# bailuding/rails

Hardware: AMD Instinct MI355X
Metric: queries/sec, MoL exact top-k over N items (get_top_k_outputs: score + top-k' + id map + seen-id filter) (higher is better)
Workload: dtype f32

## Files before the change

rails_amd/csrc/topk.hip:

```cpp
#include <hip/hip_runtime.h>
#include <stdlib.h>

#include "mol_kernels.h"

namespace mol {

constexpr int kSortCap = 16384;
constexpr int kSortThreads = 1024;
constexpr int kHistThreads = 512;
constexpr int kRadixPasses = 3;
constexpr int kBins = 2048;
__device__ __constant__ int kPassShift[kRadixPasses] = {53, 42, 32};
__device__ __constant__ int kPassBits[kRadixPasses] = {11, 11, 10};

struct SelectState {
  unsigned long long prefix;
  unsigned int need;
  unsigned int done;
  unsigned int count;
  unsigned int pad;
};

__device__ __forceinline__ unsigned int orderable(float f) {
  const unsigned int u = __float_as_uint(f);
// ... 1373 lines not shown
  if (f_invalid && !(k_out <= kFuseMaxK && f_width >= 0 && f_width <= kFuseMaxW && f_k > 0 && f_k <= k_out)) {
    set_error("merge_candidates: the seen-id filter cannot be fused at k = %d, width = %d", k_out, f_width);
    return kErrUnsupported;
  }
  const int64_t count = (int64_t)R * k;
  if (count > kSortCap) { set_error("merge_candidates: R*k = %lld exceeds the in-LDS sort capacity (%d)", (long long)count, kSortCap); return kErrUnsupported; }
  if (ensure_sort_lds() != kOk) return kErrLaunch;
  static DynLdsOnce once;
  if (ensure_dyn_lds(once, reinterpret_cast<const void*>(&merge_candidates_kernel), kSortCap * (int)sizeof(unsigned long long)) != kOk)
    return kErrLaunch;
  const int npad = next_pow2((int)count < 2 ? 2 : (int)count);
  MergeVerdictArgs v{};
  int msg_ld = 2 * k;
  if (verdict) {
    v.default_eps = verdict->default_eps; v.safety = verdict->safety; v.guard = verdict->guard; v.guard_per_row = verdict->guard ? verdict->guard_per_row : 0;
    v.guard_limit = verdict->guard_limit; v.state = verdict->state; v.state_host = verdict->state_host; v.call = verdict->call;
    msg_ld = 2 * k + 2;
  }
  hipLaunchKernelGGL(merge_candidates_kernel, dim3(rows), dim3(kSortThreads), npad * sizeof(unsigned long long), stream, gathered, R,
                     rows, k, k_out, npad, out_scores, out_ids, f_invalid, f_width, f_k, msg_ld, v);
  return hipGetLastError() == hipSuccess ? kOk : kErrLaunch;
}

__global__ __launch_bounds__(kSortThreads) void rescore_select_kernel(const float* __restrict__ exact, int64_t ld,
                                                                      const float* __restrict__ approx,
                                                                      const float* __restrict__ approx_dense, int64_t ld_dense,
                                                                      const int64_t* __restrict__ positions,
                                                                      const int64_t* __restrict__ ids, int n_ranked, int kc, int k, int npad,
                                                                      float margin_eps, float check_eps, int one_sided, float* __restrict__ out_scores,
                                                                      int64_t* __restrict__ out_ids, int* __restrict__ ok,
                                                                      float* __restrict__ stats) {
  extern __shared__ __attribute__((aligned(16))) unsigned long long keys[];
  __shared__ float red_min[kSortThreads / 64], red_err[kSortThreads / 64];
  __shared__ int red_nan[kSortThreads / 64];
  const int row = blockIdx.x;
  float mn = INFINITY, err = 0.0f;
  int bad = 0;
  for (int i = threadIdx.x; i < npad; i += kSortThreads) {
    unsigned long long kv = 0ull;
    if (i < kc) {
      const float e = exact[(int64_t)row * ld + i];
      const int64_t pos = positions[(int64_t)row * kc + i];
      float a;
      if (i < n_ranked) {
        a = approx[(int64_t)row * n_ranked + i];
        kv = ((unsigned long long)orderable(e) << 32) | (unsigned int)(~(unsigned int)pos);
        mn = fminf(mn, a);
      } else {
        a = approx_dense[(int64_t)row * ld_dense + pos];
      }
      const float dd = one_sided ? e - a : fabsf(e - a);
      bad |= !(dd <= check_eps);
      err = fmaxf(err, dd == dd ? dd : INFINITY);
    }
    keys[i] = kv;
  }
#pragma unroll
  for (int o = 32; o > 0; o >>= 1) {
    mn = fminf(mn, __shfl_xor(mn, o, 64));
    err = fmaxf(err, __shfl_xor(err, o, 64));
    bad |= __shfl_xor(bad, o, 64);
  }
  if ((threadIdx.x & 63) == 0) { red_min[threadIdx.x >> 6] = mn; red_err[threadIdx.x >> 6] = err; red_nan[threadIdx.x >> 6] = bad; }
  __syncthreads();
  for (int size = 2; size <= npad; size <<= 1) {
    for (int stride = size >> 1; stride > 0; stride >>= 1) {
      for (int t = threadIdx.x; t < (npad >> 1); t += kSortThreads) {
        const int lo = ((t & ~(stride - 1)) << 1) | (t & (stride - 1));
        const int hi2 = lo | stride;
        const bool desc = ((lo & size) == 0);
        const unsigned long long a = keys[lo], b = keys[hi2];
        if ((a < b) == desc) { keys[lo] = b; keys[hi2] = a; }
      }
      __syncthreads();
    }
  }
  for (int j = threadIdx.x; j < k; j += kSortThreads) {
    const unsigned long long kv = keys[j];
    const int64_t pos = (int64_t)(~(unsigned int)(kv & 0xFFFFFFFFull));
    out_scores[(int64_t)row * k + j] = unorderable((unsigned int)(kv >> 32));
    out_ids[(int64_t)row * k + j] = ids ? ids[pos] : pos;
  }
  if (threadIdx.x == 0) {
    float m = INFINITY, er = 0.0f;
    int b = 0;
    for (int w = 0; w < kSortThreads / 64; ++w) { m = fminf(m, red_min[w]); er = fmaxf(er, red_err[w]); b |= red_nan[w]; }
    const float kth = unorderable((unsigned int)(keys[k - 1] >> 32));
    if (ok) ok[row] = (!b && kth > m + margin_eps) ? 1 : 0;
    if (stats) { stats[2 * row] = er; stats[2 * row + 1] = kth - m; }
  }
}

__global__ __launch_bounds__(256) void rescore_verdict_kernel(const float* __restrict__ row_stats, int rows, float default_eps, float safety,
                                                              const float* __restrict__ guard, int64_t guard_count, float guard_limit,
                                                              float* __restrict__ state) {
  __shared__ float s_err[256], s_gap[256], s_grd[256];
  __shared__ int s_bad[256];
  float err = 0.0f, gap = INFINITY, grd = 0.0f;
  int bad = 0;
  for (int r = threadIdx.x; r < rows; r += 256) {
    const float e = row_stats[2 * r], g = row_stats[2 * r + 1];
    if (!(e == e) || !(g == g)) bad = 1;
    err = fmaxf(err, e);
    gap = fminf(gap, g);
  }
  for (int64_t i = threadIdx.x; i < guard_count; i += 256) {
    const float v = fabsf(guard[i]);
    if (!(v <= guard_limit)) bad = 1;
    grd = fmaxf(grd, v == v ? v : INFINITY);
  }
  s_err[threadIdx.x] = err; s_gap[threadIdx.x] = gap; s_bad[threadIdx.x] = bad; s_grd[threadIdx.x] = grd;
  __syncthreads();
  for (int w = 128; w > 0; w >>= 1) {
    if ((int)threadIdx.x < w) {
      s_err[threadIdx.x] = fmaxf(s_err[threadIdx.x], s_err[threadIdx.x + w]);
      s_gap[threadIdx.x] = fminf(s_gap[threadIdx.x], s_gap[threadIdx.x + w]);
      s_grd[threadIdx.x] = fmaxf(s_grd[threadIdx.x], s_grd[threadIdx.x + w]);
      s_bad[threadIdx.x] |= s_bad[threadIdx.x + w];
    }
    __syncthreads();
  }
  if (threadIdx.x == 0) {
    err = s_err[0]; gap = s_gap[0]; bad = s_bad[0] || !(err < INFINITY);
    float seen = state[0];
    if (!bad) seen = fmaxf(seen, err);
    const float eps = fmaxf(default_eps, safety * seen);
    const int redo = bad || !(gap > eps);
    state[0] = seen;
    reinterpret_cast<int32_t*>(state)[1] = redo;
    state[2] = eps;
    state[3] = bad ? INFINITY : err;
    state[4] = gap;
    state[5] += 1.0f;
    if (redo) state[6] += 1.0f;
    state[7] = fmaxf(state[7], s_grd[0]);
  }
}

int rescore_verdict(const float* row_stats, int rows, float default_eps, float safety, const float* guard, int64_t guard_count, float guard_limit,
                    float* state, hipStream_t stream) {
  hipLaunchKernelGGL(rescore_verdict_kernel, dim3(1), dim3(256), 0, stream, row_stats, rows, default_eps, safety, guard, guard ? guard_count : 0,
                     guard_limit, state);
  return hipGetLastError() == hipSuccess ? kOk : kErrLaunch;
}

__global__ void margin_stats_kernel(const float* __restrict__ kth, int64_t ld, int col, const float* __restrict__ m_max, const float* __restrict__ err_max,
                                    int rows, float* __restrict__ row_stats) {
  const int r = blockIdx.x * blockDim.x + threadIdx.x;
  if (r >= rows) return;
  row_stats[2 * r] = err_max[0];
  row_stats[2 * r + 1] = kth[(int64_t)r * ld + col] - m_max[r];
}
int margin_stats(const float* kth, int64_t ld, int col, const float* m_max, const float* err_max, int rows, float* row_stats, hipStream_t stream) {
  if (rows <= 0) return kOk;
  hipLaunchKernelGGL(margin_stats_kernel, dim3((rows + 255) / 256), dim3(256), 0, stream, kth, ld, col, m_max, err_max, rows, row_stats);
  return hipGetLastError() == hipSuccess ? kOk : kErrLaunch;
}

int rescore_select(const float* exact, int64_t ld, const float* approx, const float* approx_dense, int64_t ld_dense, const int64_t* positions,
                   const int64_t* ids, int rows, int n_ranked, int kc, int k, float margin_eps, float check_eps, int one_sided, float* out_scores,
                   int64_t* out_ids, int* ok, float* stats, hipStream_t stream) {
  if (rows <= 0) return kOk;
  if (kc > kSortCap) { set_error("rescore_select: %d candidates exceed the in-LDS sort capacity (%d)", kc, kSortCap); return kErrUnsupported; }
  static DynLdsOnce once;
  if (ensure_dyn_lds(once, reinterpret_cast<const void*>(&rescore_select_kernel), kSortCap * (int)sizeof(unsigned long long)) != kOk)
    return kErrLaunch;
  const int npad = next_pow2(kc < 2 ? 2 : kc);
  hipLaunchKernelGGL(rescore_select_kernel, dim3(rows), dim3(kSortThreads), npad * sizeof(unsigned long long), stream, exact, ld, approx,
                     approx_dense, ld_dense, positions, ids, n_ranked, kc, k, npad, margin_eps, check_eps, one_sided, out_scores, out_ids, ok, stats);
  return hipGetLastError() == hipSuccess ? kOk : kErrLaunch;
}

__global__ __launch_bounds__(kSortThreads) void sort_rows_i64_kernel(const int64_t* __restrict__ in, int n, int npad,
                                                                    int64_t* __restrict__ out) {
  extern __shared__ __attribute__((aligned(16))) unsigned long long keys[];
  const int row = blockIdx.x;
  if (npad >= 2 * kSortThreads && npad <= 16 * kSortThreads) {
    for (int i = threadIdx.x; i < npad; i += kSortThreads)
      keys[i] = i < n ? ~((unsigned long long)in[(int64_t)row * n + i] ^ 0x8000000000000000ull) : 0ull;
    __syncthreads();
    if (npad == 2 * kSortThreads) block_sort_desc_multi<2>(keys);
    else if (npad == 4 * kSortThreads) block_sort_desc_multi<4>(keys);
    else if (npad == 8 * kSortThreads) block_sort_desc_multi<8>(keys);
    else block_sort_desc_multi<16>(keys);
    for (int i = threadIdx.x; i < n; i += kSortThreads) out[(int64_t)row * n + i] = (int64_t)(~keys[i] ^ 0x8000000000000000ull);
    return;
  }
  for (int i = threadIdx.x; i < npad; i += kSortThreads)
    keys[i] = i < n ? ((unsigned long long)in[(int64_t)row * n + i] ^ 0x8000000000000000ull) : ~0ull;
  __syncthreads();
  for (int size = 2; size <= npad; size <<= 1) {
    for (int stride = size >> 1; stride > 0; stride >>= 1) {
      for (int t = threadIdx.x; t < (npad >> 1); t += kSortThreads) {
        const int lo = ((t & ~(stride - 1)) << 1) | (t & (stride - 1));
        const int hi2 = lo | stride;
        const bool asc = ((lo & size) == 0);
        const unsigned long long a = keys[lo], b = keys[hi2];
        if ((a > b) == asc) { keys[lo] = b; keys[hi2] = a; }
      }
      __syncthreads();
    }
  }
  for (int i = threadIdx.x; i < n; i += kSortThreads) out[(int64_t)row * n + i] = (int64_t)(keys[i] ^ 0x8000000000000000ull);
}

__global__ void mask_sorted_duplicates_kernel(const int64_t* __restrict__ idx, float* __restrict__ scores, int64_t ld,
                                              int rows, int n, float fill) {
  const int64_t i = (int64_t)blockIdx.x * blockDim.x + threadIdx.x;
  if (i >= (int64_t)rows * n) return;
  const int row = (int)(i / n), j = (int)(i - (int64_t)row * n);
  if (j > 0 && idx[i] == idx[i - 1]) scores[(int64_t)row * ld + j] = fill;
}

int sort_rows_i64(const int64_t* in, int rows, int n, int64_t* out, hipStream_t stream) {
  if (rows <= 0 || n <= 0) return kOk;
  if (n > kSortCap) { set_error("sort_rows_i64: n = %d exceeds the in-LDS sort capacity (%d)", n, kSortCap); return kErrUnsupported; }
  static DynLdsOnce once;
  if (ensure_dyn_lds(once, reinterpret_cast<const void*>(&sort_rows_i64_kernel), kSortCap * (int)sizeof(unsigned long long)) != kOk)
    return kErrLaunch;
  const int npad = next_pow2(n < 2 ? 2 : n);
  hipLaunchKernelGGL(sort_rows_i64_kernel, dim3(rows), dim3(kSortThreads), npad * sizeof(unsigned long long), stream, in, n, npad, out);
  return hipGetLastError() == hipSuccess ? kOk : kErrLaunch;
}

int mask_sorted_duplicates(const int64_t* idx, float* scores, int64_t ld, int rows, int n, float fill, hipStream_t stream) {
  const int64_t total = (int64_t)rows * n;
  if (total <= 0) return kOk;
  hipLaunchKernelGGL(mask_sorted_duplicates_kernel, dim3((unsigned)((total + 255) / 256)), dim3(256), 0, stream, idx, scores, ld, rows, n, fill);
  return hipGetLastError() == hipSuccess ? kOk : kErrLaunch;
}

constexpr int kRerankHash = 16384;
constexpr int kRerankMax = 8192;

__global__ __launch_bounds__(1024) void rerank_keys_kernel(const float* __restrict__ scores, int64_t ld, const int64_t* __restrict__ positions, int n,
                                                          int min_unique, unsigned long long* __restrict__ keys, int32_t* __restrict__ flag) {
  extern __shared__ unsigned int rr_tab[];
  const int row = blockIdx.x, tid = threadIdx.x;
  for (int i = tid; i <= kRerankHash; i += 1024) rr_tab[i] = i < kRerankHash ? 0xFFFFFFFFu : 0u;
  __syncthreads();
  unsigned int uniq = 0u;
  for (int c = tid; c < n; c += 1024) {
    const unsigned int p = (unsigned int)positions[(int64_t)row * n + c];
    unsigned int h = (p * 2654435761u) >> 18;
    bool first;
    for (;;) {
      const unsigned int old = atomicCAS(&rr_tab[h], 0xFFFFFFFFu, p);
      if (old == 0xFFFFFFFFu) { first = true; break; }
      if (old == p) { first = false; break; }
      h = (h + 1u) & (unsigned int)(kRerankHash - 1);
    }
    keys[(int64_t)row * n + c] = first ? make_key(scores[(int64_t)row * ld + c], p) : 0ull;
    uniq += first ? 1u : 0u;
  }
#pragma unroll
  for (int o = 32; o > 0; o >>= 1) uniq += (unsigned int)__shfl_xor((int)uniq, o, 64);
  if ((tid & 63) == 0 && uniq) atomicAdd(&rr_tab[kRerankHash], uniq);
  __syncthreads();
  if (tid == 0 && rr_tab[kRerankHash] < (unsigned int)min_unique) *flag = 1;
}

size_t rerank_workspace_bytes(int rows, int n_cand) { return sizeof(unsigned long long) * (size_t)rows * (size_t)n_cand; }

int rerank_topk_filtered(const float* scores, int64_t ld, int rows, int n_cand, int k_prime, const int64_t* positions, const int64_t* ids,
                         const int64_t* invalid, int width, int k, void* ws, size_t ws_bytes, int64_t* out_ids, float* out_scores, int32_t* flag,
                         hipStream_t stream) {
  if (rows <= 0 || k <= 0) return kOk;
  if (n_cand <= 1024 || n_cand > kRerankMax || !topk_can_fuse_filter(n_cand, k_prime, width, k) || k_prime > n_cand) {
    set_error("rerank_topk_filtered: unsupported size (n_cand = %d, k' = %d, width = %d, k = %d)", n_cand, k_prime, width, k);
    return kErrUnsupported;
  }
  if (ws_bytes < rerank_workspace_bytes(rows, n_cand)) { set_error("rerank_topk_filtered: workspace too small"); return kErrNoMem; }
  if (ensure_sort_lds() != kOk) return kErrLaunch;
  static DynLdsOnce once;
  const int lds = (kRerankHash + 16) * (int)sizeof(unsigned int);
  if (ensure_dyn_lds(once, reinterpret_cast<const void*>(&rerank_keys_kernel), lds) != kOk) return kErrLaunch;
  unsigned long long* keys = static_cast<unsigned long long*>(ws);
  hipLaunchKernelGGL(rerank_keys_kernel, dim3(rows), dim3(1024), lds, stream, scores, ld, positions, n_cand, k_prime, keys, flag);
  if (hipGetLastError() != hipSuccess) return kErrLaunch;
  RowSelectArgs b{};
  b.keys_in = keys; b.keys_per_row = n_cand; b.k = k_prime;
  b.ids = ids; b.ids_row_stride = 0; b.out_scores = out_scores; b.out_ids = out_ids;
  b.f_invalid = invalid; b.f_width = width; b.f_k = k;
  return launch_row_select<true>(b, rows, 1, n_cand, stream);
}

int filter_seen(const int64_t* top_ids, const float* top_scores, int rows, int k_prime, const int64_t* invalid,
                int width, int k, int64_t* out_ids, float* out_scores, hipStream_t stream) {
  if (rows <= 0) return kOk;
  if (k > k_prime) { set_error("seen-id filter: k (%d) > k' (%d)", k, k_prime); return kErrInvalid; }
  const size_t lds = sizeof(int64_t) * (size_t)width + (size_t)k_prime + 16;
  if (lds > 60000) { set_error("seen-id filter: k' or width too large for LDS"); return kErrUnsupported; }
  if (k_prime > 1024)
    hipLaunchKernelGGL(filter_seen_kernel<1024>, dim3(rows), dim3(1024), lds, stream, top_ids, top_scores, k_prime, invalid, width, k, out_ids, out_scores);
  else
    hipLaunchKernelGGL(filter_seen_kernel<256>, dim3(rows), dim3(256), lds, stream, top_ids, top_scores, k_prime, invalid, width, k, out_ids, out_scores);
  return hipGetLastError() == hipSuccess ? kOk : kErrLaunch;
}

constexpr int kCandBins = 4096, kCandCoarse = 64, kCandPer = kCandBins / kCandCoarse;
constexpr int kCandThreads = 512;
constexpr int kCandSingleMax = 65536;
constexpr int kCandStage = 2048;

struct CandWs { unsigned int* counts; unsigned int* flags; unsigned int* call; unsigned int* coarse; unsigned int* fine; };
static size_t cand_rows_pad(int rows) { return ((size_t)rows + 3) / 4 * 4; }
static size_t cand_ws_words(int rows) { return cand_rows_pad(rows) * 2 + 8 + (size_t)rows * 4 + (size_t)rows * kCandCoarse + (size_t)rows * kCandBins; }
static CandWs cand_ws(void* ws, int rows) {
  unsigned int* w = static_cast<unsigned int*>(ws);
  const size_t rp = cand_rows_pad(rows);
  CandWs c;
  c.counts = w; c.flags = w + rp; c.call = w + 2 * rp; c.coarse = c.call + 8 + 4 * (size_t)rows; c.fine = c.coarse + (size_t)rows * kCandCoarse;
  return c;
}
size_t candidates_workspace_bytes(int rows) { return cand_ws_words(rows < 1 ? 1 : rows) * sizeof(unsigned int); }

__device__ __forceinline__ int cand_bin(float s, float lo, float scale) {
  float x = (s - lo) * scale;
  x = fminf(fmaxf(x, 0.0f), (float)(kCandBins - 1));
  return (int)x;
}

template <int NT, class F4, class F1>
__device__ __forceinline__ void walk_chunk4(const float* __restrict__ rowp, int64_t begin, int64_t end, F4 f4, F1 f1) {
  int64_t a0 = begin + ((4 - (int64_t)((reinterpret_cast<uintptr_t>(rowp + begin) >> 2) & 3)) & 3);
  if (a0 > end) a0 = end;
  const int64_t nvec = (end - a0) >> 2;
  for (int64_t i = begin + threadIdx.x; i < a0; i += NT) f1(rowp[i], i);
  const float4* body = reinterpret_cast<const float4*>(rowp + a0);
  int64_t v = threadIdx.x;
  for (; v + 3 * NT < nvec; v += 4 * NT) {
    const float4 x0 = body[v], x1 = body[v + NT], x2 = body[v + 2 * NT], x3 = body[v + 3 * NT];
    f4(x0, a0 + 4 * v); f4(x1, a0 + 4 * (v + NT)); f4(x2, a0 + 4 * (v + 2 * NT)); f4(x3, a0 + 4 * (v + 3 * NT));
  }
  for (; v < nvec; v += NT) f4(body[v], a0 + 4 * v);
  for (int64_t i = a0 + 4 * nvec + threadIdx.x; i < end; i += NT) f1(rowp[i], i);
}

__device__ __forceinline__ float cand_threshold_value(int bt, float lo, float scale) {
  if (bt <= 0) return -INFINITY;
  if (cand_bin(INFINITY, lo, scale) < bt) return __uint_as_float(0x7FC00000u);
  if (cand_bin(-INFINITY, lo, scale) >= bt) return -INFINITY;
  unsigned int a = orderable(-INFINITY), b = orderable(INFINITY);
  while (b - a > 1u) {
    const unsigned int mid = a + ((b - a) >> 1);
    if (cand_bin(unorderable(mid), lo, scale) >= bt) b = mid; else a = mid;
  }
  return unorderable(b);
}

template <int NT>
__device__ __forceinline__ void cand_coarse_sums(const unsigned int* h, unsigned int* hc) {
  constexpr int run = kCandBins / NT;
  constexpr int per = kCandPer / run;
  unsigned int s = 0u;
#pragma unroll
  for (int j = 0; j < run; ++j) s += h[threadIdx.x * run + j];
#pragma unroll
  for (int o = 1; o < per; o <<= 1) s += __shfl_xor(s, o, 64);
  if ((threadIdx.x & (per - 1)) == 0) hc[threadIdx.x / per] = s;
}

__device__ __forceinline__ int cand_pick(const unsigned int* coarse, const unsigned int* fine, unsigned int cap, int lane) {
  const unsigned int cc = coarse[kCandCoarse - 1 - lane];
  unsigned int incl = cc;
#pragma unroll
  for (int o = 1; o < 64; o <<= 1) { const unsigned int v = __shfl_up(incl, o, 64); if (lane >= o) incl += v; }
  const unsigned long long over = __ballot(incl > cap);
  if (over == 0ull) return 0;
  const int first = __ffsll((long long)over) - 1;
  const int cg = kCandCoarse - 1 - first;
  const unsigned int base = (unsigned int)__shfl((int)(incl - cc), first, 64);
  const unsigned int f = fine[cg * kCandPer + kCandPer - 1 - lane];
  unsigned int incl2 = f;
#pragma unroll
  for (int o = 1; o < 64; o <<= 1) { const unsigned int v = __shfl_up(incl2, o, 64); if (lane >= o) incl2 += v; }
  const int fit = __popcll(__ballot(base + incl2 <= cap));
  return cg * kCandPer + kCandPer - fit;
}

template <int NT>
__device__ __forceinline__ void cand_append(const float* __restrict__ rowp, int64_t begin, int64_t end, float thr,
                                            unsigned int* count, int64_t* __restrict__ out_pos, float* __restrict__ out_a, unsigned int cap,
                                            unsigned long long* stage, unsigned int* wg_base, unsigned int* wg_cursor) {
  const int lane = threadIdx.x & 63;
  if (threadIdx.x == 0) *wg_cursor = 0u;
  __syncthreads();
  auto put = [&](bool sel, float sc, int64_t i, unsigned int base_all, bool direct) {
    const unsigned long long m = __ballot(sel);
    if (m) {
      const int leader = __ffsll((long long)m) - 1;
      unsigned int base = 0;
      if (lane == leader) base = atomicAdd(wg_cursor, (unsigned int)__popcll(m));
      base = (unsigned int)__shfl((int)base, leader, 64);
      if (sel) {
        const unsigned int slot = base + (unsigned int)__popcll(m & ((1ull << lane) - 1ull));
        if (!direct) { if (slot < (unsigned int)kCandStage) stage[slot] = ((unsigned long long)__float_as_uint(sc) << 32) | (unsigned int)i; }
        else if (base_all + slot < cap) { out_pos[base_all + slot] = i; out_a[base_all + slot] = sc; }
      }
    }
  };
  auto walk = [&](unsigned int base_all, bool direct) {
    walk_chunk4<NT>(rowp, begin, end,
        [&](const float4 x, int64_t i) {
          const bool s0 = x.x >= thr, s1 = x.y >= thr, s2 = x.z >= thr, s3 = x.w >= thr;
          if (__ballot(s0 | s1 | s2 | s3) != 0ull) {
            put(s0, x.x, i, base_all, direct); put(s1, x.y, i + 1, base_all, direct); put(s2, x.z, i + 2, base_all, direct); put(s3, x.w, i + 3, base_all, direct);
          }
        },
        [&](float sc, int64_t i) { put(sc >= thr, sc, i, base_all, direct); });
  };
  walk(0u, false);
  __syncthreads();
  const unsigned int total = *wg_cursor;
  if (total == 0u) return;
  __syncthreads();
  if (threadIdx.x == 0) { *wg_base = atomicAdd(count, total); *wg_cursor = 0u; }
  __syncthreads();
  const unsigned int wbase = *wg_base;
  if (total <= (unsigned int)kCandStage) {
    for (unsigned int j = threadIdx.x; j < total; j += NT) {
      const unsigned long long e = stage[j];
      if (wbase + j < cap) { out_pos[wbase + j] = (int64_t)(unsigned int)e; out_a[wbase + j] = __uint_as_float((unsigned int)(e >> 32)); }
    }
    return;
  }
  walk(wbase, true);
}

__global__ __launch_bounds__(kCandThreads) void cand_hist_kernel(const float* __restrict__ scores, int64_t ld, int64_t n, int64_t chunk, float lo,
                                                                float scale, unsigned int cap, CandWs w) {
  __shared__ __attribute__((aligned(16))) unsigned int h[kCandBins];
  __shared__ unsigned int hc[kCandCoarse];
  __shared__ int s_cut;
  const int row = blockIdx.y, tid = threadIdx.x, lane = tid & 63;
  for (int i = tid; i < kCandBins; i += kCandThreads) h[i] = 0u;
  __syncthreads();
  const int64_t begin = (int64_t)blockIdx.x * chunk;
  const int64_t end = (begin + chunk < n) ? begin + chunk : n;
  const float* rowp = scores + (int64_t)row * ld;
  bool nan = false;
  auto one = [&](float sc, int64_t) { nan |= !(sc == sc); atomicAdd(&h[cand_bin(sc, lo, scale)], 1u); };
  walk_chunk4<kCandThreads>(rowp, begin, end, [&](const float4 x, int64_t i) { one(x.x, i); one(x.y, i); one(x.z, i); one(x.w, i); }, one);
  if (__ballot(nan) != 0ull && lane == 0) atomicOr(&w.flags[row], 1u);
  __syncthreads();
  cand_coarse_sums<kCandThreads>(h, hc);
  __syncthreads();
  if (tid < 64) {
    const unsigned int cc = hc[kCandCoarse - 1 - lane];
    unsigned int incl = cc;
#pragma unroll
    for (int o = 1; o < 64; o <<= 1) { const unsigned int v = __shfl_up(incl, o, 64); if (lane >= o) incl += v; }
    const unsigned long long over = __ballot(incl > cap);
    if (lane == 0) s_cut = over ? kCandCoarse - 1 - (__ffsll((long long)over) - 1) : 0;
  }
  __syncthreads();
  const int cut = s_cut;
  unsigned int* gf = w.fine + (size_t)row * kCandBins;
  unsigned int* gc = w.coarse + (size_t)row * kCandCoarse;
  for (int i = cut * kCandPer + tid; i < kCandBins; i += kCandThreads)
    if (h[i]) atomicAdd(&gf[i], h[i]);
  if (tid < kCandCoarse && tid >= cut && hc[tid]) atomicAdd(&gc[tid], hc[tid]);
}

__global__ __launch_bounds__(kCandThreads) void cand_compact_kernel(const float* __restrict__ scores, int64_t ld, int64_t n, int64_t chunk, float lo,
                                                                   float scale, unsigned int cap, CandWs w, int64_t* __restrict__ out_pos,
                                                                   float* __restrict__ out_a, int64_t cand_ld) {
  __shared__ unsigned long long stage[kCandStage];
  __shared__ unsigned int wg_base, wg_cursor;
  __shared__ float s_thr;
  const int row = blockIdx.y, tid = threadIdx.x;
  if (tid < 64) {
    const int bt = cand_pick(w.coarse + (size_t)row * kCandCoarse, w.fine + (size_t)row * kCandBins, cap, tid);
    if (tid == 0) s_thr = cand_threshold_value(bt, lo, scale);
  }
  __syncthreads();
  const int64_t begin = (int64_t)blockIdx.x * chunk;
  const int64_t end = (begin + chunk < n) ? begin + chunk : n;
  cand_append<kCandThreads>(scores + (int64_t)row * ld, begin, end, s_thr, &w.counts[row], out_pos + (int64_t)row * cand_ld,
                            out_a + (int64_t)row * cand_ld, cap, stage, &wg_base, &wg_cursor);
}

__global__ __launch_bounds__(kRowThreads) void cand_single_kernel(const float* __restrict__ scores, int64_t ld, int64_t n, float lo, float scale,
                                                                 unsigned int cap, CandWs w, int64_t* __restrict__ out_pos, float* __restrict__ out_a,
                                                                 int64_t cand_ld) {
  __shared__ __attribute__((aligned(16))) unsigned int h[kCandBins];
  __shared__ unsigned int hc[kCandCoarse];
  __shared__ unsigned long long stage[kCandStage];
  __shared__ unsigned int wg_base, wg_cursor;
  __shared__ float s_thr;
  const int row = blockIdx.x, tid = threadIdx.x, lane = tid & 63;
  for (int i = tid; i < kCandBins; i += kRowThreads) h[i] = 0u;
  __syncthreads();
  const float* rowp = scores + (int64_t)row * ld;
  bool nan = false;
  auto one = [&](float sc, int64_t) { nan |= !(sc == sc); atomicAdd(&h[cand_bin(sc, lo, scale)], 1u); };
  walk_chunk4<kRowThreads>(rowp, 0, n, [&](const float4 x, int64_t i) { one(x.x, i); one(x.y, i); one(x.z, i); one(x.w, i); }, one);
  if (__ballot(nan) != 0ull && lane == 0) atomicOr(&w.flags[row], 1u);
  __syncthreads();
  cand_coarse_sums<kRowThreads>(h, hc);
  __syncthreads();
  if (tid < 64) {
    const int bt = cand_pick(hc, h, cap, tid);
    if (tid == 0) s_thr = cand_threshold_value(bt, lo, scale);
  }
  __syncthreads();
  cand_append<kRowThreads>(rowp, 0, n, s_thr, &w.counts[row], out_pos + (int64_t)row * cand_ld, out_a + (int64_t)row * cand_ld, cap, stage,
                           &wg_base, &wg_cursor);
}

int candidates_select(const float* scores, int64_t ld, int rows, int64_t n, int cap, float lo, float hi, void* ws, int64_t* out_pos, float* out_approx,
                      int64_t cand_ld, int n_cu, hipStream_t stream) {
  if (rows <= 0 || n <= 0) return kOk;
  if (cap < 1 || cap > kSortCap || cand_ld < cap) { set_error("candidates_select: cap = %d out of range (1 .. %d, row stride %lld)", cap, kSortCap, (long long)cand_ld); return kErrInvalid; }
  if (n >= (1ll << 32)) { set_error("candidates_select: n = %lld does not fit 32-bit positions", (long long)n); return kErrUnsupported; }
  if (!(hi > lo)) { set_error("candidates_select: empty score range"); return kErrInvalid; }
  const float scale = (float)kCandBins / (hi - lo);
  const CandWs w = cand_ws(ws, rows);
  if (n <= kCandSingleMax) {
    hipLaunchKernelGGL(cand_single_kernel, dim3(rows), dim3(kRowThreads), 0, stream, scores, ld, n, lo, scale, (unsigned int)cap, w, out_pos, out_approx, cand_ld);
    return hipGetLastError() == hipSuccess ? kOk : kErrLaunch;
  }
  const int target = 2 * (n_cu > 0 ? n_cu : 256);
  int64_t chunks = (target + rows - 1) / rows;
  const int64_t max_chunks = (n + 8191) / 8192;
  if (chunks > max_chunks) chunks = max_chunks;
  if (chunks < 1) chunks = 1;
  int64_t chunk = (n + chunks - 1) / chunks;
  chunk = (chunk + 3) / 4 * 4;
  chunks = (n + chunk - 1) / chunk;
  hipLaunchKernelGGL(cand_hist_kernel, dim3((unsigned)chunks, rows), dim3(kCandThreads), 0, stream, scores, ld, n, chunk, lo, scale, (unsigned int)cap, w);
  hipLaunchKernelGGL(cand_compact_kernel, dim3((unsigned)chunks, rows), dim3(kCandThreads), 0, stream, scores, ld, n, chunk, lo, scale, (unsigned int)cap, w,
                     out_pos, out_approx, cand_ld);
  return hipGetLastError() == hipSuccess ? kOk : kErrLaunch;
}

struct CandFinishArgs {
  const float* exact; int64_t ld;
  const float* approx; const int64_t* pos; int64_t cand_ld;
  CandWs w; int cap, npad, k;
  const int64_t* ids; int64_t n_items;
  float default_eps, safety; int one_sided;
  const float* guard; int guard_per_row; float guard_limit;
  float* out_scores; int64_t* out_ids;
  const int64_t* f_invalid; int f_width, f_k; int64_t* f_out_ids; float* f_out_scores;
  float* state; float* state_host;
  int clean_hist;
  int64_t* msg;
};

__global__ __launch_bounds__(kSortThreads) void cand_finish_kernel(const CandFinishArgs a) {
  extern __shared__ __attribute__((aligned(16))) unsigned long long keys[];
  __shared__ float red_min[kSortThreads / 64], red_err[kSortThreads / 64], red_grd[kSortThreads / 64];
  __shared__ int red_bad[kSortThreads / 64];
  __shared__ int64_t f_id[kFuseMaxK], f_inv[kFuseMaxW];
  __shared__ float f_sc[kFuseMaxK];
  __shared__ int f_scratch[kSortThreads / 64 + 2];
  __shared__ int s_last;
  const int row = blockIdx.x, rows = gridDim.x, tid = threadIdx.x, lane = tid & 63;
  const int k = a.k, npad = a.npad;
  const bool fuse = a.f_invalid != nullptr;
  const unsigned int flags = a.w.flags[row];
  const float seen_before = a.state ? a.state[0] : 0.0f;
  if (fuse)
    for (int i = tid; i < a.f_width; i += kSortThreads) f_inv[i] = a.f_invalid[(int64_t)row * a.f_width + i];
  float mn = INFINITY, err = 0.0f, grd = 0.0f;
  int bad = (flags & 1u) ? 1 : 0;
  unsigned int c = a.w.counts[row];
  if (c > (unsigned int)a.cap) c = (unsigned int)a.cap;
  for (int i = tid; i < npad; i += kSortThreads) {
    unsigned long long kv = 0ull;
    float e = 0.0f, ap = 0.0f;
    int64_t p = 0;
    if (i < a.cap) {
      e = a.exact[(int64_t)row * a.ld + i];
      ap = a.approx[(int64_t)row * a.cand_ld + i];
      p = a.pos[(int64_t)row * a.cand_ld + i];
    }
    if (i < (int)c) {
      kv = ((unsigned long long)orderable(e) << 32) | (unsigned int)(~(unsigned int)p);
      mn = fminf(mn, ap);
      const float dd = a.one_sided ? fmaxf(e - ap, 0.0f) : fabsf(e - ap);
      bad |= !(dd == dd) || !(e == e) || !(ap == ap);
      err = fmaxf(err, dd == dd ? dd : INFINITY);
    }
    keys[i] = kv;
  }
  if (a.guard)
    for (int i = tid; i < a.guard_per_row; i += kSortThreads) {
      const float v = fabsf(a.guard[(int64_t)row * a.guard_per_row + i]);
      if (!(v <= a.guard_limit)) bad = 1;
      grd = fmaxf(grd, v == v ? v : INFINITY);
    }
#pragma unroll
  for (int o = 32; o > 0; o >>= 1) {
    mn = fminf(mn, __shfl_xor(mn, o, 64));
    err = fmaxf(err, __shfl_xor(err, o, 64));
    grd = fmaxf(grd, __shfl_xor(grd, o, 64));
    bad |= __shfl_xor(bad, o, 64);
  }
  if (lane == 0) { red_min[tid >> 6] = mn; red_err[tid >> 6] = err; red_grd[tid >> 6] = grd; red_bad[tid >> 6] = bad; }
  {
    if (a.clean_hist) {
      unsigned int* gf = a.w.fine + (size_t)row * kCandBins;
      for (int i = tid; i < kCandBins; i += kSortThreads) gf[i] = 0u;
      if (tid < kCandCoarse) a.w.coarse[(size_t)row * kCandCoarse + tid] = 0u;
    }
    if (tid == 0) { a.w.counts[row] = 0u; a.w.flags[row] = 0u; }
  }
  __syncthreads();
  if (npad <= kSortThreads) {
    unsigned long long kv = tid < npad ? keys[tid] : 0ull;
    kv = block_sort_desc(kv, npad, keys + npad);
    __syncthreads();
    if (tid < npad) keys[tid] = kv;
    __syncthreads();
  } else if (npad == 2 * kSortThreads) block_sort_desc_multi<2>(keys);
  else if (npad == 4 * kSortThreads) block_sort_desc_multi<4>(keys);
  else if (npad == 8 * kSortThreads) block_sort_desc_multi<8>(keys);
  else block_sort_desc_multi<16>(keys);
  mn = INFINITY; err = 0.0f; grd = 0.0f; bad = 0;
  for (int wv = 0; wv < kSortThreads / 64; ++wv) { mn = fminf(mn, red_min[wv]); err = fmaxf(err, red_err[wv]); grd = fmaxf(grd, red_grd[wv]); bad |= red_bad[wv]; }
  const bool whole_row = (int64_t)c >= a.n_items;
  if (whole_row) mn = -INFINITY;
  else if (c == 0u) mn = INFINITY;
  if (a.msg) {
    int64_t* m = a.msg + (int64_t)row * (2 * k + 2);
    for (int j = tid; j < k; j += kSortThreads) {
      const unsigned long long kv = j < (int)c ? keys[j] : 0ull;
      const int64_t p = (int64_t)(~(unsigned int)(kv & 0xFFFFFFFFull));
      const float sc = kv ? unorderable((unsigned int)(kv >> 32)) : -INFINITY;
      m[j] = (int64_t)(unsigned long long)__float_as_uint(sc);
      m[k + j] = kv ? (a.ids ? a.ids[p] : p) : -1;
    }
    if (tid == 0) {
      m[2 * k] = (int64_t)(unsigned long long)__float_as_uint(mn);
      m[2 * k + 1] = (int64_t)(unsigned long long)__float_as_uint(bad ? INFINITY : err);
    }
    return;
  }
  for (int j = tid; j < k; j += kSortThreads) {
    const unsigned long long kv = keys[j];
    const int64_t p = (int64_t)(~(unsigned int)(kv & 0xFFFFFFFFull));
    const float sc = unorderable((unsigned int)(kv >> 32));
    const int64_t id = a.ids ? a.ids[p < a.n_items ? p : 0] : p;
    a.out_scores[(int64_t)row * k + j] = sc;
    a.out_ids[(int64_t)row * k + j] = id;
    if (fuse && j < kFuseMaxK) { f_sc[j] = sc; f_id[j] = id; }
  }
  const float kth = (int)c >= k ? unorderable((unsigned int)(keys[k - 1] >> 32)) : -INFINITY;
  const float gap = kth - mn;
  const float eps = fmaxf(a.default_eps, a.safety * fmaxf(seen_before, bad ? 0.0f : err));
  const int fail = bad || (int)c < k || !(gap > eps);
  if (fuse) {
    __syncthreads();
    filter_from_lds<kSortThreads>(f_id, f_sc, k, f_inv, a.f_width, a.f_k, a.f_out_ids + (int64_t)row * a.f_k, a.f_out_scores + (int64_t)row * a.f_k, f_scratch);
  }
  verdict_commit(a.w.call, row, rows, fail, bad, err, gap, grd, a.default_eps, a.safety, a.state, a.state_host, &s_last);
}

int candidates_finish(const float* exact, int64_t ld, const float* approx, const int64_t* pos, int64_t cand_ld, int cap, void* ws, const int64_t* ids,
                      int64_t n_items, int rows, int k, float default_eps, float safety, int one_sided, const float* guard, int guard_per_row,
                      float guard_limit, float* out_scores, int64_t* out_ids, const int64_t* f_invalid, int f_width, int f_k, int64_t* f_out_ids,
                      float* f_out_scores, float* state, float* state_host, int64_t* msg, hipStream_t stream) {
  if (rows <= 0) return kOk;
  if (cap < 1 || cap > kSortCap || k < 1 || (k > cap && !msg)) { set_error("candidates_finish: k = %d of cap = %d out of range", k, cap); return kErrInvalid; }
  if (f_invalid && !(k <= kFuseMaxK && f_width >= 0 && f_width <= kFuseMaxW && f_k > 0 && f_k <= k)) {
    set_error("candidates_finish: the seen-id filter cannot be fused at k = %d, width = %d", k, f_width);
    return kErrUnsupported;
  }
  static DynLdsOnce once;
  if (ensure_dyn_lds(once, reinterpret_cast<const void*>(&cand_finish_kernel), kSortCap * (int)sizeof(unsigned long long)) != kOk) return kErrLaunch;
  CandFinishArgs a{};
  a.exact = exact; a.ld = ld; a.approx = approx; a.pos = pos; a.cand_ld = cand_ld; a.w = cand_ws(ws, rows); a.cap = cap; a.k = k;
  int npad = next_pow2(cap < 64 ? 64 : cap);
  a.npad = npad;
  a.ids = ids; a.n_items = n_items; a.default_eps = default_eps; a.safety = safety; a.one_sided = one_sided;
  a.guard = guard; a.guard_per_row = guard ? guard_per_row : 0; a.guard_limit = guard_limit;
  a.out_scores = out_scores; a.out_ids = out_ids;
  a.f_invalid = f_invalid; a.f_width = f_width; a.f_k = f_k; a.f_out_ids = f_out_ids; a.f_out_scores = f_out_scores;
  a.state = state; a.state_host = state_host; a.msg = msg;
  a.clean_hist = n_items > kCandSingleMax ? 1 : 0;
  const size_t lds = (size_t)(npad <= kSortThreads ? 3 * npad : npad) * sizeof(unsigned long long);
  hipLaunchKernelGGL(cand_finish_kernel, dim3(rows), dim3(kSortThreads), lds, stream, a);
  return hipGetLastError() == hipSuccess ? kOk : kErrLaunch;
}

}
```

Measured before the change: 12210.

## Fuse candidate histogram and compaction into one register-held single-pass kernel

Adds a fused candidate-selection kernel that loads each chunk into registers once, builds the local histogram, writes a per-chunk candidate list using a local threshold, and lets the last-arriving block per row compute the global threshold and compact the lists. This replaces the separate histogram and compact launches, which read the scores twice, with a single read and a single launch. It adds a larger workspace for per-chunk lists, last-block serialization per row, and heavier register pressure from holding the data. The old two-kernel path is kept as a fallback when the size limits are not met.

```diff
diff --git a/rails_amd/csrc/topk.hip b/rails_amd/csrc/topk.hip
--- a/rails_amd/csrc/topk.hip
+++ b/rails_amd/csrc/topk.hip
@@ -1699,15 +1699,29 @@
 constexpr int kCandThreads = 512;
 constexpr int kCandSingleMax = 65536;
 constexpr int kCandStage = 2048;
-
-struct CandWs { unsigned int* counts; unsigned int* flags; unsigned int* call; unsigned int* coarse; unsigned int* fine; };
+constexpr int kCandHoldVec = 12;
+constexpr int kCandHold = kCandHoldVec * 4 * kRowThreads;
+constexpr int kCandListGroups = 512;
+constexpr int kCandListSlot = 1024;
+constexpr int kCandMaxChunks = kCandBins;
+
+struct CandWs {
+  unsigned int* counts; unsigned int* flags; unsigned int* call; unsigned int* coarse; unsigned int* fine;
+  unsigned int* arrive; unsigned int* lcount; unsigned long long* lists;
+};
 static size_t cand_rows_pad(int rows) { return ((size_t)rows + 3) / 4 * 4; }
-static size_t cand_ws_words(int rows) { return cand_rows_pad(rows) * 2 + 8 + (size_t)rows * 4 + (size_t)rows * kCandCoarse + (size_t)rows * kCandBins; }
+static size_t cand_ws_head_words(int rows) { return cand_rows_pad(rows) * 2 + 8 + (size_t)rows * 4 + (size_t)rows * kCandCoarse + (size_t)rows * kCandBins; }
+static size_t cand_list_entries(int rows) { return ((size_t)kCandListGroups + (size_t)rows) * kCandListSlot; }
+static size_t cand_ws_words(int rows) {
+  return cand_ws_head_words(rows) + cand_rows_pad(rows) + ((size_t)kCandListGroups + cand_rows_pad(rows)) + 2 * cand_list_entries(rows);
+}
 static CandWs cand_ws(void* ws, int rows) {
   unsigned int* w = static_cast<unsigned int*>(ws);
   const size_t rp = cand_rows_pad(rows);
   CandWs c;
   c.counts = w; c.flags = w + rp; c.call = w + 2 * rp; c.coarse = c.call + 8 + 4 * (size_t)rows; c.fine = c.coarse + (size_t)rows * kCandCoarse;
+  c.arrive = w + cand_ws_head_words(rows); c.lcount = c.arrive + rp;
+  c.lists = reinterpret_cast<unsigned long long*>(c.lcount + kCandListGroups + rp);
   return c;
 }
 size_t candidates_workspace_bytes(int rows) { return cand_ws_words(rows < 1 ? 1 : rows) * sizeof(unsigned int); }
@@ -1774,6 +1788,14 @@
   for (int o = 1; o < 64; o <<= 1) { const unsigned int v = __shfl_up(incl2, o, 64); if (lane >= o) incl2 += v; }
   const int fit = __popcll(__ballot(base + incl2 <= cap));
   return cg * kCandPer + kCandPer - fit;
+}
+
+__device__ __forceinline__ int cand_cut(const unsigned int* hc, unsigned int cap, int lane) {
+  unsigned int incl = hc[kCandCoarse - 1 - lane];
+#pragma unroll
+  for (int o = 1; o < 64; o <<= 1) { const unsigned int v = __shfl_up(incl, o, 64); if (lane >= o) incl += v; }
+  const unsigned long long over = __ballot(incl > cap);
+  return over ? kCandCoarse - 1 - (__ffsll((long long)over) - 1) : 0;
 }
 
 template <int NT>
@@ -1844,12 +1866,8 @@
   cand_coarse_sums<kCandThreads>(h, hc);
   __syncthreads();
   if (tid < 64) {
-    const unsigned int cc = hc[kCandCoarse - 1 - lane];
-    unsigned int incl = cc;
-#pragma unroll
-    for (int o = 1; o < 64; o <<= 1) { const unsigned int v = __shfl_up(incl, o, 64); if (lane >= o) incl += v; }
-    const unsigned long long over = __ballot(incl > cap);
-    if (lane == 0) s_cut = over ? kCandCoarse - 1 - (__ffsll((long long)over) - 1) : 0;
+    const int c = cand_cut(hc, cap, lane);
+    if (lane == 0) s_cut = c;
   }
   __syncthreads();
   const int cut = s_cut;
@@ -1876,6 +1894,148 @@
   const int64_t end = (begin + chunk < n) ? begin + chunk : n;
   cand_append<kCandThreads>(scores + (int64_t)row * ld, begin, end, s_thr, &w.counts[row], out_pos + (int64_t)row * cand_ld,
                             out_a + (int64_t)row * cand_ld, cap, stage, &wg_base, &wg_cursor);
+}
+
+__global__ __launch_bounds__(kRowThreads) void cand_fused_kernel(const float* __restrict__ scores, int64_t ld, int64_t n, int64_t chunk, float lo,
+                                                                float scale, unsigned int cap, CandWs w, unsigned int slot,
+                                                                int64_t* __restrict__ out_pos, float* __restrict__ out_a, int64_t cand_ld) {
+  __shared__ __attribute__((aligned(16))) unsigned int h[kCandBins];
+  __shared__ unsigned int hc[kCandCoarse];
+  __shared__ unsigned int s_cursor;
+  __shared__ int s_cut, s_last;
+  __shared__ float s_thr;
+  const int row = blockIdx.y, tid = threadIdx.x, lane = tid & 63;
+  const unsigned int chunks = gridDim.x;
+  for (int i = tid; i < kCandBins; i += kRowThreads) h[i] = 0u;
+  if (tid == 0) s_cursor = 0u;
+  const int64_t begin = (int64_t)blockIdx.x * chunk;
+  const int64_t end = (begin + chunk < n) ? begin + chunk : n;
+  const float* rowp = scores + (int64_t)row * ld;
+  int64_t a0 = begin + ((4 - (int64_t)((reinterpret_cast<uintptr_t>(rowp + begin) >> 2) & 3)) & 3);
+  if (a0 > end) a0 = end;
+  const int nvec = (int)((end - a0) >> 2);
+  const float4* body = reinterpret_cast<const float4*>(rowp + a0);
+  float4 v[kCandHoldVec];
+#pragma unroll
+  for (int j = 0; j < kCandHoldVec; ++j) {
+    v[j] = float4{0.0f, 0.0f, 0.0f, 0.0f};
+    if (j * kRowThreads + tid < nvec) v[j] = body[j * kRowThreads + tid];
+  }
+  int64_t epos = -1;
+  if (tid < 64) { if (begin + tid < a0) epos = begin + tid; }
+  else if (tid < 128) { const int64_t p = a0 + 4 * (int64_t)nvec + (tid - 64); if (p < end) epos = p; }
+  const bool edge = epos >= 0;
+  const float ev = edge ? rowp[epos] : 0.0f;
+  __syncthreads();
+  bool nan = false;
+  auto one = [&](float sc) { nan |= !(sc == sc); atomicAdd(&h[cand_bin(sc, lo, scale)], 1u); };
+#pragma unroll
+  for (int j = 0; j < kCandHoldVec; ++j)
+    if (j * kRowThreads + tid < nvec) { one(v[j].x); one(v[j].y); one(v[j].z); one(v[j].w); }
+  if (edge) one(ev);
+  if (__ballot(nan) != 0ull && lane == 0) atomicOr(&w.flags[row], 1u);
+  __syncthreads();
+  cand_coarse_sums<kRowThreads>(h, hc);
+  __syncthreads();
+  if (tid < 64) {
+    const int cut = cand_cut(hc, cap, lane);
+    const int bl = cand_pick(hc, h, cap, lane);
+    if (lane == 0) { s_cut = cut; s_thr = cand_threshold_value(bl, lo, scale); }
+  }
+  __syncthreads();
+  {
+    const int cut = s_cut;
+    unsigned int* gf = w.fine + (size_t)row * kCandBins;
+    unsigned int* gc = w.coarse + (size_t)row * kCandCoarse;
+    for (int i = cut * kCandPer + tid; i < kCandBins; i += kRowThreads)
+      if (h[i]) atomicAdd(&gf[i], h[i]);
+    if (tid < kCandCoarse && tid >= cut && hc[tid]) atomicAdd(&gc[tid], hc[tid]);
+  }
+  const size_t group = (size_t)row * chunks + blockIdx.x;
+  unsigned long long* list = w.lists + group * slot;
+  {
+    const float thr = s_thr;
+    unsigned int mine = edge && ev >= thr ? 1u : 0u;
+#pragma unroll
+    for (int j = 0; j < kCandHoldVec; ++j)
+      if (j * kRowThreads + tid < nvec) mine += (v[j].x >= thr ? 1u : 0u) + (v[j].y >= thr ? 1u : 0u) + (v[j].z >= thr ? 1u : 0u) + (v[j].w >= thr ? 1u : 0u);
+    unsigned int incl = mine;
+#pragma unroll
+    for (int o = 1; o < 64; o <<= 1) { const unsigned int u = __shfl_up(incl, o, 64); if (lane >= o) incl += u; }
+    unsigned int base = 0u;
+    if (lane == 63 && incl) base = atomicAdd(&s_cursor, incl);
+    base = (unsigned int)__shfl((int)base, 63, 64);
+    unsigned int at = base + incl - mine;
+    auto put = [&](float sc, int64_t i) {
+      if (sc >= thr) { if (at < slot) list[at] = ((unsigned long long)__float_as_uint(sc) << 32) | (unsigned int)i; ++at; }
+    };
+    if (mine) {
+#pragma unroll
+      for (int j = 0; j < kCandHoldVec; ++j)
+        if (j * kRowThreads + tid < nvec) {
+          const int64_t i = a0 + 4 * (int64_t)(j * kRowThreads + tid);
+          put(v[j].x, i); put(v[j].y, i + 1); put(v[j].z, i + 2); put(v[j].w, i + 3);
+        }
+      if (edge) put(ev, epos);
+    }
+  }
+  __threadfence();
+  __syncthreads();
+  if (tid == 0) {
+    const unsigned int total = s_cursor < slot ? s_cursor : slot;
+    if (total) w.lcount[group] = total;
+    __threadfence();
+    s_last = atomicAdd(&w.arrive[row], 1u) == chunks - 1u ? 1 : 0;
+  }
+  __syncthreads();
+  if (!s_last) return;
+  __threadfence();
+  unsigned int* s_cnt = h;
+  {
+    volatile unsigned int* lc = w.lcount + (size_t)row * chunks;
+    for (unsigned int c = tid; c < chunks; c += kRowThreads) { s_cnt[c] = lc[c]; lc[c] = 0u; }
+  }
+  if (tid < 64) {
+    const int bt = cand_pick(w.coarse + (size_t)row * kCandCoarse, w.fine + (size_t)row * kCandBins, cap, tid);
+    if (tid == 0) { s_thr = cand_threshold_value(bt, lo, scale); s_cursor = 0u; }
+  }
+  __syncthreads();
+  {
+    const float thr = s_thr;
+    unsigned long long* rl = w.lists + (size_t)row * chunks * slot;
+    int64_t* op = out_pos + (int64_t)row * cand_ld;
+    float* oa = out_a + (int64_t)row * cand_ld;
+    const unsigned int all = chunks * slot;
+    constexpr int kAhead = 4;
+    for (unsigned int b0 = 0u; b0 < all; b0 += kAhead * kRowThreads) {
+      unsigned long long e[kAhead];
+      bool ok[kAhead];
+#pragma unroll
+      for (int u = 0; u < kAhead; ++u) {
+        const unsigned int idx = b0 + u * kRowThreads + tid;
+        const unsigned int c = idx / slot;
+        ok[u] = idx < all && idx - c * slot < s_cnt[c];
+        e[u] = 0ull;
+        if (ok[u]) { e[u] = rl[idx]; rl[idx] = 0ull; }
+      }
+#pragma unroll
+      for (int u = 0; u < kAhead; ++u) {
+        const float sc = __uint_as_float((unsigned int)(e[u] >> 32));
+        const bool sel = ok[u] && sc >= thr;
+        const unsigned long long m = __ballot(sel);
+        if (m) {
+          const int leader = __ffsll((long long)m) - 1;
+          unsigned int base = 0u;
+          if (lane == leader) base = atomicAdd(&s_cursor, (unsigned int)__popcll(m));
+          base = (unsigned int)__shfl((int)base, leader, 64);
+          const unsigned int at = base + (unsigned int)__popcll(m & ((1ull << lane) - 1ull));
+          if (sel && at < cap) { op[at] = (int64_t)(unsigned int)e[u]; oa[at] = sc; }
+        }
+      }
+    }
+  }
+  __syncthreads();
+  if (tid == 0) { w.counts[row] = s_cursor < cap ? s_cursor : cap; w.arrive[row] = 0u; }
 }
 
 __global__ __launch_bounds__(kRowThreads) void cand_single_kernel(const float* __restrict__ scores, int64_t ld, int64_t n, float lo, float scale,
@@ -1919,6 +2079,25 @@
     return hipGetLastError() == hipSuccess ? kOk : kErrLaunch;
   }
   const int target = 2 * (n_cu > 0 ? n_cu : 256);
+  {
+    const int64_t per_list = cap < n ? cap : n;
+    int64_t chunks = ((target < kCandListGroups ? target : kCandListGroups) + rows - 1) / rows;
+    const int64_t max_chunks = (n + 8191) / 8192, fit = (int64_t)(cand_list_entries(rows) / ((size_t)rows * (size_t)per_list));
+    const int64_t need = (n + kCandHold - 1) / kCandHold;
+    if (chunks > max_chunks) chunks = max_chunks;
+    if (chunks > fit) chunks = fit;
+    if (chunks < need) chunks = need;
+    int64_t chunk = (n + chunks - 1) / chunks;
+    chunk = (chunk + 3) / 4 * 4;
+    chunks = (n + chunk - 1) / chunk;
+    const int64_t slot = cap < chunk ? cap : chunk;
+    if (chunk <= kCandHold && chunks <= kCandMaxChunks && (int64_t)rows * chunks <= (int64_t)kCandListGroups + rows &&
+        (size_t)rows * (size_t)chunks * (size_t)slot <= cand_list_entries(rows)) {
+      hipLaunchKernelGGL(cand_fused_kernel, dim3((unsigned)chunks, rows), dim3(kRowThreads), 0, stream, scores, ld, n, chunk, lo, scale, (unsigned int)cap, w,
+                         (unsigned int)slot, out_pos, out_approx, cand_ld);
+      return hipGetLastError() == hipSuccess ? kOk : kErrLaunch;
+    }
+  }
   int64_t chunks = (target + rows - 1) / rows;
   const int64_t max_chunks = (n + 8191) / 8192;
   if (chunks > max_chunks) chunks = max_chunks;
```

Result: slower. 10970 (-10.2%).
